# yjxiong/action-detection

Measured on AMD Instinct MI355X. Metric: proposals/sec (9-seg BNInception SSN fwd+bwd), higher is better.
Workload: dtype f32

## Files before the change

action-detection_amd/_lib.py:

```python
import ctypes
import os
import subprocess
import threading

import torch

_HERE = os.path.dirname(os.path.abspath(__file__))
CSRC = os.path.join(_HERE, "csrc")
LIB_PATH = os.path.join(_HERE, "libssn_hip.so")
SOURCES = ["conv_igemm.hip", "conv_x6.hip", "conv_x6_rect.hip", "conv_wgrad.hip", "conv_wgrad_x6.hip", "elementwise.hip", "bn_train.hip", "frames.hip", "detect.hip", "detect_batch.hip", "pool.hip", "stpp.hip", "heads_losses.hip", "conv_pl.hip", "planes_ops.hip", "planes_bn.hip", "wgrad_pl.hip", "tag.hip", "eval.hip", "actionness.hip", "train_step.hip", "flow.hip", "jpeg.hip", "jpeg_encode.hip", "jpeg_transcode.hip", "jpeg_roundtrip.hip", "video_cls.hip", "proposal_list.hip", "proposal_text.hip", "proposal_eval.hip", "test_table.hip"]

STPP_MAX_PARTS = 24


class SsnStppTable(ctypes.Structure):
    _fields_ = [("n_parts", ctypes.c_int), ("n_seg", ctypes.c_int),
                ("act_lo", ctypes.c_int), ("act_hi", ctypes.c_int),
                ("lo", ctypes.c_int * STPP_MAX_PARTS), ("hi", ctypes.c_int * STPP_MAX_PARTS),
                ("norm", ctypes.c_int * STPP_MAX_PARTS), ("col", ctypes.c_int * STPP_MAX_PARTS)]


_SIGS = {
    "ssn_conv_bn_relu_fwd": "pppppiiiiliiiliiiiipp",
    "ssn_bn_fold": "pppppfppip",
    "ssn_relu_bn_bwd": "pppiiillpp",
    "ssn_conv_dgrad": "pppiiiiliiiliiiiplpiipp",
    "ssn_conv_pack_weights": "ppiiiip",
    "ssn_conv_pack_weights_multi": "ippppppppp",
    "ssn_conv_wgrad": "ppppiiiiliiiliiiplip",
    "ssn_conv_wgrad_x6": "ppppiiiililiiiplippiipp",
    "ssn_wgrad_reduce": "pppiiip",
    "ssn_wgrad_reduce_taps": "pppiiiip",
    "ssn_conv_x6_pack_weights_multi": "ippppppppppppp",
    "ssn_conv_x6_fwd": "pppppiiiiliiiliiiiiippiiipp",
    "ssn_conv_x6_dgrad": "pppiiiiliiiliiiplpiippiipp",
    "ssn_conv_x6_fwd_rect": "pppppiiiiliiiliiiiiiippp",
    "ssn_conv_x6_pack_dgrad_s2": "ppiip",
    "ssn_conv_x6_dgrad_s2": "pppiiiiliiiliplpiippip",
    "ssn_conv_x6_pack_dgrad_rect": "ppiiiip",
    "ssn_conv_x6_pack_rect_multi": "ipppppppp",
    "ssn_conv_x6_dgrad_rect": "pppiiiililiiiiiplpiippp",
    "ssn_conv_wgrad_x6_rect": "ppppiiiililiiiiiplippp",
    "ssn_conv_x6_pack_weights_rect": "ppiiiip",
# ... 75 lines not shown
    "ssn_row_scatter": "pppiiip",
    "ssn_ce_loss_fwd": "ppppiip",
    "ssn_ce_loss_bwd": "pppppiip",
    "ssn_completeness_loss_fwd": "pppppiiiiiifp",
    "ssn_completeness_loss_bwd": "ppppiifp",
    "ssn_cw_smoothl1_fwd": "pppppiip",
    "ssn_total_loss_fwd": "ppiippiiiiiifpppiiffpppppp",
    "ssn_total_loss_bwd": "ppiipiifpiiffpppppppp",
    "ssn_label_select": "pppipipippppp",
    "ssn_param_checksum": "pipppip",
    "ssn_cw_smoothl1_bwd": "ppppiip",
    "ssn_sgd_step": "ppplffffipp",
    "ssn_sgd_step_multi": "ippppppffipp",
    "ssn_bn_fold_multi": "ipppppppppp",
    "ssn_sumsq": "plpipp",
    "ssn_step_meters": "plpiipidppp",
    "ssn_sumsq_multi": "ippplffpp",
    "ssn_sgd_step_multi_dev": "ippppppfpipp",
    "ssn_scale": "plpfp",
    "ssn_add_inplace": "pplp",
    "ssn_embed_planes": "ppiiiiliilp",
    "ssn_space_to_depth2": "ppiiiipp",
    "ssn_s2d_weights": "ppiiip",
    "ssn_s2d_weights_bwd": "ppiiip",
    "ssn_pl_scales_update": "pppiiiip",
    "ssn_pl_range_check": "pppiip",
    "ssn_pl_from_f32": "plppiiiilippp",
    "ssn_pl_to_f32": "pplpliiipp",
    "ssn_pl_im2col": "pplppliiiiiiiiiiip",
    "ssn_conv_pl_fwd": "pppppppiiiiliiiliiiiiiipppiiip",
    "ssn_conv_pl_dgrad": "pppppiiiiliiiliiiiiplpipppiiip",
    "ssn_conv_wgrad_pl": "ppppppiiiiliiiliiiiiplippiipp",
    "ssn_wgrad_reduce_multi": "ipppppppp",
    "ssn_conv_wgrad_pl_group": "ippppppppppplplp",
    "ssn_conv_wgrad_pl_group_lanes": "ippppppppppplplp" + "pii",
    "ssn_conv_pl_dgrad_s2": "pppppiiiiliiiliiplpipppp",
    "ssn_pl_maxpool_fwd": "pplpplpiiiiiiiiipppp",
    "ssn_pl_maxpool_bwd": "pplpppl" + "i" * 10 + "plpipppplp",
    "ssn_pl_avgpool_affine": "pplpplppiiiiiiipppp",
    "ssn_pl_relu_bn_bwd": "pplplpiiippp",
    "ssn_pl_gap_fwd": "pplpiiipp",
    "ssn_pl_gap_bwd": "pppliiiplpppp",
    "ssn_pl_channel_sum": "pplpiiipplp",
    "ssn_pl_channel_sum_multi": "ippppipppplp",
    "ssn_conv_x6_pack_batch_begin": "",
    "ssn_conv_x6_pack_batch_end": "plip",
    "ssn_conv_x6_pack_batch_end_lanes": "pliipp",
    "ssn_conv_x6_pack_batch_join": "p",
    "ssn_pl_bn_train_stats": "pplpppppp" + "iiiffplp",
    "ssn_pl_bn_train_apply": "pplppplpp" + "ppppiiiip",
    "ssn_pl_bn_train_bwd": "pplpplpplp" + "ppppp" + "pplpp" + "pliiiplp",
}
_CT = {"p": ctypes.c_void_p, "i": ctypes.c_int, "l": ctypes.c_long, "f": ctypes.c_float, "d": ctypes.c_double,
       "u": ctypes.c_ulonglong}

EXPORTS = sorted(list(_SIGS) + ["ssn_last_error", "ssn_abi_version", "ssn_conv_wgrad_workspace_bytes",
                                "ssn_conv_pick_tile", "ssn_conv_packed_floats", "ssn_conv_x6_packed_floats", "ssn_conv_x6_packed_floats_rect", "ssn_conv_x6_packed_floats_dgrad_rect", "ssn_conv_wgrad_x6_rect_workspace_bytes", "ssn_conv_x6_dgrad_s2_packed_floats", "ssn_conv_x6_debug_flags", "ssn_conv_x6_debug_trace",
                                "ssn_conv_wgrad_x6_workspace_bytes", "ssn_detections_workspace_bytes", "ssn_detections_batch_workspace_bytes",
                                "ssn_conv_debug_flags", "ssn_channel_sum_shares", "ssn_bn_train_workspace_floats",
                                "ssn_conv_dgrad_layout", "ssn_conv_pl_tiles", "ssn_conv_pl_halo_taken", "ssn_conv_pl_debug_flags", "ssn_conv_pl_debug_trace", "ssn_conv_wgrad_pl_debug_trace", "ssn_conv_wgrad_pl_debug_flags", "ssn_conv_pl_tile_shape", "ssn_conv_wgrad_pl_tiles", "ssn_conv_wgrad_pl_workspace_bytes", "ssn_conv_wgrad_pl_group_workspace_bytes", "ssn_conv_wgrad_pl_group_table_bytes", "ssn_conv_wgrad_pl_group_tuning", "ssn_pl_channel_sum_workspace_bytes", "ssn_pl_bn_train_workspace_bytes", "ssn_conv_x6_pack_batch_entries", "ssn_conv_x6_pack_entry_bytes", "ssn_conv_x6_pack_batch_abort", "ssn_frames_resize_workspace_bytes", "ssn_frames_scale_workspace_bytes",
                                "ssn_tag_workspace_bytes", "ssn_tag_lds_candidates", "ssn_eval_workspace_bytes", "ssn_eval_lds_gt",
                                "ssn_proposal_eval_max_points", "ssn_proposal_eval_workspace_bytes",
                                "ssn_vcls_lds_rows", "ssn_vcls_metrics_workspace_bytes",
                                "ssn_sumsq_multi_workspace_floats", "ssn_train_step_launches"])


# ... 178 lines not shown
```

action-detection_amd/csrc/wgrad_pl.hip:

```cpp
#include "planes.h"

#include <algorithm>
#include <cmath>
#include <cstdlib>
#include <map>
#include <mutex>
#include <vector>

namespace {

using namespace pl;

struct WgPlArgs {
    const void* g_hi;
    const void* g_lo;
    const void* x_hi;
    const void* x_lo;
    float* part;
    unsigned long long* trace;
    int dbg;
    const float* g_scale;
    const float* x_scale;
    int g_row_split, g_row_gap;
    int N, Cin, H, W;
// ... 484 lines not shown
        if (ci >= p.Cin) continue;
#pragma unroll
        for (int i = 0; i < TM; ++i)
#pragma unroll
            for (int r = 0; r < 16; ++r) {
                const int m = m0 + (wm * TM + i) * 32 + (r & 3) + 8 * (r >> 2) + 4 * lh;
                if (m < p.M) {
#pragma unroll
                    for (int t = 0; t < KK; ++t) out[(long)m * p.ldp + t * p.Cin + ci] = acc[t][i][j][r] * inv;
                }
            }
    }
    if (do_bias && li == 0) {
        const float ginv = 1.f / *p.g_scale;
#pragma unroll
        for (int i = 0; i < TM; ++i)
#pragma unroll
            for (int r = 0; r < 16; ++r) {
                const int m = m0 + (wm * TM + i) * 32 + (r & 3) + 8 * (r >> 2) + 4 * lh;
                if (m < p.M) out[(long)m * p.ldp + p.K] = accb[i][r] * ginv;
            }
    }
    trc.end(p);
}

template <int KK, int TM, int TC, int XP, int KG = 1>
__global__ __launch_bounds__(256 * KG, (KG > 1 || KK * TM * TC >= 18 || TM * TC >= 4) ? 1 : 2) void wgrad_pl9_kernel(WgPlArgs p) {
    __shared__ __attribute__((aligned(1024))) unsigned char lds[wgpl9_lds_bytes<TM, TC, XP>()];
    wgrad_pl9_body<KK, TM, TC, XP, KG>(p, blockIdx.x, lds);
}


constexpr int WGG_MAX = 96;
constexpr int WGG_WRITE = 12;
struct WgGroupEntry {
    WgPlArgs a;
    int variant;
    uint32_t nblk;
};
struct WgGroupIndex {
    int count;
    int blk0[WGG_MAX + 1];
};
struct WgGroupChunk {
    WgGroupEntry e[WGG_WRITE];
    int count;
};
__global__ __launch_bounds__(64) void wgrad_group_write_kernel(WgGroupChunk c, WgGroupEntry* table, int first) {
    if ((int)threadIdx.x < c.count) table[first + threadIdx.x] = c.e[threadIdx.x];
}
__device__ __forceinline__ int group_problem_of_block(const WgGroupIndex& ix, int b) {
    int lo = 0, hi = ix.count - 1;
    while (lo < hi) {
        const int mid = (lo + hi + 1) >> 1;
        if (ix.blk0[mid] <= b) lo = mid; else hi = mid - 1;
    }
    return wave_uniform(lo);
}

template <int XP, int KG, int KH = 3, int KW = 3>
__global__ __launch_bounds__(256 * KG, KG > 1 ? 1 : 2) void wgrad_group9_kernel(const WgGroupEntry* __restrict__ table, WgGroupIndex ix) {
    __shared__ __attribute__((aligned(1024))) unsigned char lds[wgpl9_lds_bytes<1, 1, XP>()];
    const int e = group_problem_of_block(ix, (int)blockIdx.x);
    const uint32_t bid = blockIdx.x - (uint32_t)ix.blk0[e];
    const auto* ent = SSN_CONST_PTR(WgGroupEntry, table) + e;
    if (bid >= ent->nblk) return;
    const WgPlArgs p = ent->a;
    wgrad_pl9_body<KH * KW, 1, 1, XP, KG, KH, KW, KH / 2, KW / 2>(p, bid, lds);
}

constexpr int WGG1_LDS = 65536;
static_assert(wgpl_lds_dwords<2, 2, 2, 2>() * 4 <= WGG1_LDS && wgpl_lds_dwords<1, 4, 3, 1>() * 4 <= WGG1_LDS &&
              wgpl_lds_dwords<2, 2, 1, 1>() * 4 <= WGG1_LDS && wgpl9_lds_bytes<1, 1, 4>() <= WGG1_LDS, "group LDS");
__global__ __launch_bounds__(256, 2) void wgrad_group1_kernel(const WgGroupEntry* __restrict__ table, WgGroupIndex ix) {
    __shared__ __attribute__((aligned(1024))) unsigned char lds[WGG1_LDS];
    const int e = group_problem_of_block(ix, (int)blockIdx.x);
    const uint32_t bid = blockIdx.x - (uint32_t)ix.blk0[e];
    const auto* ent = SSN_CONST_PTR(WgGroupEntry, table) + e;
    if (bid >= ent->nblk) return;
    const WgPlArgs p = ent->a;
// ... 631 lines not shown
    for (WgGroupItem& it : items) {
        it.ws_off = off;
        off += ((long)it.a.splits * it.kg * it.a.M * it.a.ldp * (long)sizeof(float) + 1023) / 1024 * 1024;
    }
    *ws_total = off;
    return SSN_OK;
}
}

extern "C" void ssn_conv_wgrad_pl_group_tuning(double fixed_nine, double fixed_one, int min_units_nine, int min_units_one) {
    if (fixed_nine > 0) g_group_fixed[0] = fixed_nine;
    if (fixed_one > 0) g_group_fixed[1] = fixed_one;
    if (min_units_nine > 0) g_group_min_units[0] = min_units_nine;
    if (min_units_one > 0) g_group_min_units[1] = min_units_one;
}
extern "C" long ssn_conv_wgrad_pl_group_table_bytes(int count) { return (long)(count > 0 ? count : 1) * (long)sizeof(WgGroupEntry); }

extern "C" long ssn_conv_wgrad_pl_group_workspace_bytes(int count, const int* shape, const long* groups, int* plan_out) {
    if (count <= 0 || !shape || !groups) return 0;
    std::vector<WgGroupItem> items;
    long total = 0;
    if (plan_group_all(count, shape, groups, nullptr, nullptr, nullptr, nullptr, nullptr, nullptr, nullptr, nullptr, items, &total) != SSN_OK)
        return -1;
    if (plan_out)
        for (int i = 0; i < count; ++i) {
            plan_out[i * 4] = items[(size_t)i].family;
            plan_out[i * 4 + 1] = items[(size_t)i].variant;
            plan_out[i * 4 + 2] = items[(size_t)i].a.splits;
            plan_out[i * 4 + 3] = items[(size_t)i].a.ksteps_per_split;
        }
    return total;
}

extern "C" int ssn_wgrad_reduce_multi(int count, const float* const* part, float* const* dw, float* const* db, const int* M,
                                      const int* K, const int* splits, const int* taps, hipStream_t stream);

namespace {
constexpr int WGL_MAX = 8;
#if defined(__HIP__)
struct WgLaneEvents {
    hipEvent_t fork;
    hipEvent_t join[WGL_MAX];
};
WgLaneEvents* wgrad_lane_events(hipStream_t stream) {
    static std::mutex mu;
    static std::map<int, WgLaneEvents> cache;
    std::lock_guard<std::mutex> lock(mu);
    int dev = 0;
    if (hipGetDevice(&dev) != hipSuccess) return nullptr;
    auto it = cache.find(dev);
    if (it != cache.end()) return &it->second;
    hipStreamCaptureStatus status = hipStreamCaptureStatusNone;
    if (hipStreamIsCapturing(stream, &status) != hipSuccess || status != hipStreamCaptureStatusNone) {
        (void)hipGetLastError();
        return nullptr;
    }
    WgLaneEvents ev;
    bool ok = hipEventCreateWithFlags(&ev.fork, hipEventDisableTiming) == hipSuccess;
    for (int k = 0; k < WGL_MAX && ok; ++k) ok = hipEventCreateWithFlags(&ev.join[k], hipEventDisableTiming) == hipSuccess;
    if (!ok) {
        (void)hipGetLastError();
        return nullptr;
    }
    return &cache.emplace(dev, ev).first->second;
}
#endif

int wgrad_group_run(int count, const void* const* g_hi, const void* const* g_lo, const void* const* x_hi, const void* const* x_lo,
// ... 41 lines not shown
                return ((double)x->a.M + (double)x->a.Cin * s2) / ((double)x->a.M * x->a.Cin * x->a.kh * x->a.kw);
            };
            std::stable_sort(fam.begin(), fam.end(), [&](const WgGroupItem* x, const WgGroupItem* y) { return bytes_per_mac(x) > bytes_per_mac(y); });
            std::vector<WgGroupItem*> dealt;
            for (size_t lo = 0, hi = fam.size(); lo < hi;) {
                dealt.push_back(fam[lo++]);
                if (lo < hi) dealt.push_back(fam[--hi]);
            }
            fam.swap(dealt);
        }
        for (size_t base = 0; base < fam.size(); base += WGG_MAX) {
            const int n = (int)std::min<size_t>(WGG_MAX, fam.size() - base);
            Launch L;
            L.family = f;
            L.first = first;
            L.items.assign(fam.begin() + (long)base, fam.begin() + (long)base + n);
            L.slab_bytes = 0;
            for (const WgGroupItem* it : L.items) L.slab_bytes += (long)it->a.splits * it->kg * it->a.M * it->a.ldp * (long)sizeof(float);
            launches.push_back(std::move(L));
            first += n;
        }
    }
    if (per_family)
        std::stable_sort(launches.begin(), launches.end(), [](const Launch& x, const Launch& y) { return x.slab_bytes > y.slab_bytes; });

    int fan = n_lanes;
#if defined(__HIP__)
    WgLaneEvents* ev = fan > 0 ? wgrad_lane_events(stream) : nullptr;
    if (!ev) fan = 0;
#else
    SSN_CHECK_ARG(n_lanes == 0, "conv wgrad pl group: the host build has no streams");
#endif

    auto write_table = [&](const Launch& L, WgGroupIndex& ix) -> long {
        const int n = (int)L.items.size();
        ix.count = n;
        long blocks = 0;
        for (int c0 = 0; c0 < n; c0 += WGG_WRITE) {
            WgGroupChunk ch;
            ch.count = std::min(WGG_WRITE, n - c0);
            for (int j = 0; j < ch.count; ++j) {
                WgGroupItem& it = *L.items[(size_t)(c0 + j)];
                it.a.part = reinterpret_cast<float*>(static_cast<char*>(workspace) + it.ws_off);
                ch.e[j].a = it.a;
                ch.e[j].variant = it.variant;
                ch.e[j].nblk = (uint32_t)(it.tiles * it.a.splits);
                ix.blk0[c0 + j] = (int)blocks;
                blocks += (it.tiles * it.a.splits + 7) / 8 * 8;
            }
            hipLaunchKernelGGL(wgrad_group_write_kernel, dim3(1), dim3(64), 0, stream, ch, dev, L.first + c0);
        }
        for (int j = n; j <= WGG_MAX; ++j) ix.blk0[j] = (int)blocks;
        return blocks;
    };
    auto launch_family = [&](const Launch& L, const WgGroupIndex& ix, long blocks, hipStream_t s) {
        const WgGroupEntry* tab = dev + L.first;
        switch (L.family) {
            case WGF_9_XP6: hipLaunchKernelGGL((wgrad_group9_kernel<6, 1>), dim3((unsigned)blocks), dim3(256), 0, s, tab, ix); break;
            case WGF_9_XP8: hipLaunchKernelGGL((wgrad_group9_kernel<8, 2>), dim3((unsigned)blocks), dim3(512), 0, s, tab, ix); break;
            case WGF_9_XP12: hipLaunchKernelGGL((wgrad_group9_kernel<12, 2>), dim3((unsigned)blocks), dim3(512), 0, s, tab, ix); break;
            case WGF_STEM: hipLaunchKernelGGL(wgrad_group_stem_kernel, dim3((unsigned)blocks), dim3(512), 0, s, tab, ix); break;
            case WGF_7_ROW: hipLaunchKernelGGL((wgrad_group9_kernel<6, 1, 1, 7>), dim3((unsigned)blocks), dim3(256), 0, s, tab, ix); break;
            case WGF_7_COL: hipLaunchKernelGGL((wgrad_group9_kernel<12, 2, 7, 1>), dim3((unsigned)blocks), dim3(512), 0, s, tab, ix); break;
            default: hipLaunchKernelGGL(wgrad_group1_kernel, dim3((unsigned)blocks), dim3(256), 0, s, tab, ix); break;
        }
    };
    auto reduce = [&](const std::vector<const WgGroupItem*>& its, hipStream_t s) -> int {
        const size_t n = its.size();
        std::vector<const float*> parts(n);
        std::vector<float*> dws(n), dbs(n);
        std::vector<int> Ms(n), Ks(n), sp(n), tp(n);
        for (size_t i = 0; i < n; ++i) {
            const WgGroupItem& it = *its[i];
            parts[i] = reinterpret_cast<const float*>(static_cast<char*>(workspace) + it.ws_off);
            dws[i] = it.dw;
            dbs[i] = it.db;
            Ms[i] = it.a.M;
            Ks[i] = it.a.K;
            sp[i] = it.a.splits * it.kg;
            tp[i] = it.taps;
        }
        return ssn_wgrad_reduce_multi((int)n, parts.data(), dws.data(), dbs.data(), Ms.data(), Ks.data(), sp.data(), tp.data(), s);
    };

    std::vector<WgGroupIndex> index(launches.size());
    std::vector<long> grid(launches.size());
    if (fan > 0) {
        for (size_t k = 0; k < launches.size(); ++k) {
            grid[k] = write_table(launches[k], index[k]);
            SSN_CHECK_ARG(grid[k] < (1l << 31), "conv wgrad pl group: too many blocks");
        }
        SSN_CHECK_LAUNCH("conv_wgrad_pl_group");
    }
#if defined(__HIP__)
    if (fan > 0) {
        bool ok = hipEventRecord(ev->fork, stream) == hipSuccess;
        for (int k = 0; k < fan && ok; ++k) ok = hipStreamWaitEvent(lanes[k], ev->fork, 0) == hipSuccess;
        if (!ok) {
            ssn_set_error("conv wgrad pl group: fork of the side streams failed: %s", hipGetErrorString(hipGetLastError()));
            return SSN_ERR_LAUNCH;
        }
    }
#endif
    for (size_t k = 0; k < launches.size(); ++k) {
        const Launch& L = launches[k];
        hipStream_t s = fan > 0 ? lanes[k % (size_t)fan] : stream;
        if (fan == 0) {
            grid[k] = write_table(L, index[k]);
            SSN_CHECK_ARG(grid[k] < (1l << 31), "conv wgrad pl group: too many blocks");
        }
        launch_family(L, index[k], grid[k], s);
        if (per_family) {
            SSN_CHECK_LAUNCH("conv_wgrad_pl_group");
            rc = reduce(std::vector<const WgGroupItem*>(L.items.begin(), L.items.end()), s);
            if (rc != SSN_OK) break;
        }
    }
#if defined(__HIP__)
    if (fan > 0 && join) {
        bool ok = true;
        for (int k = 0; k < fan; ++k) {
            ok = hipEventRecord(ev->join[k], lanes[k]) == hipSuccess && ok;
            ok = hipStreamWaitEvent(stream, ev->join[k], 0) == hipSuccess && ok;
        }
        if (!ok && rc == SSN_OK) {
            ssn_set_error("conv wgrad pl group: join of the side streams failed: %s", hipGetErrorString(hipGetLastError()));
            return SSN_ERR_LAUNCH;
        }
    }
#endif
    if (rc != SSN_OK) return rc;
    SSN_CHECK_LAUNCH("conv_wgrad_pl_group");
    if (per_family) return SSN_OK;
    std::vector<const WgGroupItem*> all((size_t)count);
    for (int i = 0; i < count; ++i) all[(size_t)i] = &items[(size_t)i];
    return reduce(all, stream);
}
}

extern "C" int ssn_conv_wgrad_pl_group(int count, const void* const* g_hi, const void* const* g_lo, const void* const* x_hi,
                                       const void* const* x_lo, float* const* dw, float* const* db, const int* shape,
// ... 86 lines not shown
```

action-detection_amd/planes.py:

```python
import torch

from . import _lib
from . import kernels as K
from .kernels import _p, _stream


class SlotPool:

    def __init__(self, n, device, flag=None):
        self.device = device
        self.amax = torch.zeros(n, device=device, dtype=torch.float32)
        self.scale = torch.ones(n, device=device, dtype=torch.float32)
        self.flag = torch.zeros(2, device=device, dtype=torch.int32) if flag is None else flag
        self.used = 0
        self.odd_extra_bits = 0

    def take(self):
        i = self.used
        if i >= self.amax.numel():
            raise RuntimeError("slot pool exhausted")
        self.used += 1
        return i

    def update(self, exact=False, first=0, count=None):
# ... 158 lines not shown
             mask.groups if mask is not None else 0, _p(mask_scale), tile_cfg, dy.t.scale_ptr, dx.t.scale_ptr, dx.t.amax_ptr,
             int(k_split), int(k_gap), int(bool(taps_reversed)), _st(lib, dy.t))


def wgrad_workspace_bytes(n, cin, cout, ho, wo, kh, kw, tile_cfg=-1):
    return int(_lib.get_lib().cdll.ssn_conv_wgrad_pl_workspace_bytes(n, cin, cout, ho, wo, kh, kw, tile_cfg))


def conv_wgrad(g, x, dw, db, kh, kw, stride, pad_h, pad_w, workspace, tile_cfg=-1, cin=None, g_row_split=0, g_row_gap=0, defer=None):
    import ctypes
    lib = _lib_for(g.t)
    h, w = x.hw
    ho, wo = g.hw
    cin = x.c if cin is None else cin
    info = (ctypes.c_int * 2)() if defer is not None else None
    lib.call("ssn_conv_wgrad_pl", g.hi, g.lo, x.hi, x.lo, _p(dw), _p(db), x.n, cin, h, w, x.groups, g.c, ho, wo, g.groups, kh, kw,
             stride, pad_h, pad_w, _p(workspace), workspace.numel() * workspace.element_size(), tile_cfg, g.t.scale_ptr,
             x.t.scale_ptr, int(g_row_split), int(g_row_gap), ctypes.addressof(info) if info is not None else None, _st(lib, g.t))
    if defer is not None:
        defer.append((workspace, dw, db, g.c, cin * kh * kw, int(info[0]), int(info[1])))


def wgrad_reduce_multi(entries):
    import ctypes
    if not entries:
        return
    lib = _lib.get_lib()
    n = len(entries)
    parts = (ctypes.c_void_p * n)(*[e[0].data_ptr() for e in entries])
    dws = (ctypes.c_void_p * n)(*[e[1].data_ptr() for e in entries])
    dbs = (ctypes.c_void_p * n)(*[(e[2].data_ptr() if e[2] is not None else None) for e in entries])
    arr = [(ctypes.c_int * n)(*[int(e[k]) for e in entries]) for k in (3, 4, 5, 6)]
    lib.call("ssn_wgrad_reduce_multi", n, ctypes.addressof(parts), ctypes.addressof(dws), ctypes.addressof(dbs),
             ctypes.addressof(arr[0]), ctypes.addressof(arr[1]), ctypes.addressof(arr[2]), ctypes.addressof(arr[3]),
             _stream(lib, entries[0][0]))


class WgradJob:

    __slots__ = ("g", "x", "dw", "db", "kh", "kw", "stride", "pad_h", "pad_w", "cin", "g_row_split", "g_row_gap", "hint", "units")

    def __init__(self, g, x, dw, db, kh, kw, stride, pad_h, pad_w, cin=None, g_row_split=0, g_row_gap=0, hint=-1, units=0):
        self.g, self.x, self.dw, self.db = g, x, dw, db
        self.kh, self.kw, self.stride, self.pad_h, self.pad_w = int(kh), int(kw), int(stride), int(pad_h), int(pad_w)
        self.cin = x.c if cin is None else int(cin)
        self.g_row_split, self.g_row_gap, self.hint = int(g_row_split), int(g_row_gap), int(hint)
        self.units = int(units)

    def shape16(self):
        h, w = self.x.hw
        ho, wo = self.g.hw
        return [self.x.n, self.cin, h, w, self.g.c, ho, wo, self.kh, self.kw, self.stride, self.pad_h, self.pad_w,
                self.g_row_split, self.g_row_gap, self.hint, self.units]


def _wgrad_group_arrays(jobs):
    import ctypes
    n = len(jobs)
    shape = (ctypes.c_int * (16 * n))(*[v for j in jobs for v in j.shape16()])
    groups = (ctypes.c_long * (2 * n))(*[v for j in jobs for v in (j.x.groups, j.g.groups)])
    return shape, groups


def wgrad_group_plan(jobs):
    import ctypes
    lib = _lib.get_lib()
# ... 182 lines not shown
```

action-detection_amd/planes_exec.py:

```python
import contextlib
import itertools
import math

import torch

from . import kernels as K
from . import planes as P
from .planes import PSlice, PlaneTensor


class PlanesState:

    MAX_TENSORS = 512
    GRAD_EXTRA_BITS = 3

    def __init__(self, device, flag=None):
        self.pool = P.SlotPool(2 * self.MAX_TENSORS, device, flag)
        self.pool.odd_extra_bits = self.GRAD_EXTRA_BITS
        self.act_slot = {}
        self.grad_slot = {}
        self.fwd_calibrated = False
        self.bwd_calibrated = False
        self.calibration_passes = [0, 0]
        self.recalibrations = [0, 0]
# ... 447 lines not shown
            ws_bytes = max(ws_bytes, need)
        else:
            ws_off[op["lids"][0]] = (ws_bytes, need)
            ws_bytes += need
    ws_all = net._workspace(ws_bytes, dev)

    def ws_of(op):
        if op["lids"][0] not in ws_off:
            return None
        o, nb = ws_off[op["lids"][0]]
        return ws_all[o // 4:(o + nb) // 4]
    cs_ws = torch.empty(P.channel_sum_workspace_bytes(sum(op["cout"] for op in plan if op["kind"] == "conv" and
                                                           (op.get("raw") or "raw_from" in op)) + 8) // 4,
                        device=dev, dtype=torch.float32)

    dg_s2 = {op["lids"][0]: _dgrad_is_s2(op) for op in plan if op["kind"] == "conv" and op["src"] != "data"}
    packed_dg = extras["packed_dg"]

    def src_key(op):
        return (op["src"], op.get("src_c0", 0))
    last_writer = {}
    for idx in range(len(plan) - 1, -1, -1):
        last_writer[src_key(plan[idx])] = idx
    first_conv = net._conv_ids[0]
    stem_out = None
    for op in plan:
        if op["kind"] == "conv" and op.get("s2d") and "data_s2d_f32" in acts:
            readers = [q for q in plan if q.get("src") == op["dst"]]
            if len(readers) == 1 and readers[0]["kind"] == "pool" and readers[0]["pool"] == "max" and op["dst_c0"] == 0:
                stem_out = op["dst"]

    conv_of = {op["dst"]: op for op in plan if op["kind"] == "conv" and op.get("bn_train")}

    def launch_all(grads, fire_hook):
        masked, inited = {}, set()
        pending_end = total
        pending_reduce, pending_sums = [], []

        pending_wgrad = []
        wgrad_flops_total = sum(2.0 * n * shapes[q["dst"]][1] * shapes[q["dst"]][2] * q["cout"] * q["cin"] * _conv_taps(q)[0] * _conv_taps(q)[1]
                                for q in plan if q["kind"] == "conv")
        pending_post = []

        if not (net.wgrad_lanes and net.group_wgrad):
            wl_streams = None
        elif dfeat.is_cuda and net.overlap_wgrad and net.branch_lanes:
            cur = torch.cuda.current_stream(dev).cuda_stream
            wl_streams = [s for s in net._wgrad_streams(dev, 3) if s.cuda_stream != cur]
        else:
            wl_streams = []

        def flush():
            if pending_wgrad:
                jobs = [j for j, _ in pending_wgrad]
                net._timed("conv_wgrad_pl", "group", sum(f for _, f in pending_wgrad),
                           lambda: P.conv_wgrad_group(jobs, *net._wgrad_group_buffers(jobs, dev), streams=wl_streams))
            if pending_reduce:
                entries = list(pending_reduce)
                net._timed("conv_wgrad_pl", "reduce_multi", 0.0, lambda: P.wgrad_reduce_multi(entries))
            if pending_sums:
                P.channel_sum_multi(list(pending_sums), cs_ws)
            for fn in pending_post:
                fn()
            del pending_reduce[:], pending_sums[:], pending_wgrad[:], pending_post[:]
        group = net.group_wgrad
        defer = pending_reduce if net.defer_wgrad_reduce else None

# ... 169 lines not shown
                        net._timed("conv_dgrad_pl", lids[0], flops,
                                   lambda: P.conv_dgrad_s2(gs, wt, dx, op["p"], acc_flag, tcfg, mask=my, mask_scale=ms))
                    else:
                        net._timed("conv_dgrad_pl", lids[0], flops, lambda: P.conv_dgrad(
                            gs, wt, dx, kh, kw, ph, pw, acc_flag, tcfg, mask=my, mask_scale=ms, k_split=op.get("row_split", 0),
                            k_gap=op.get("row_gap", 0), taps_reversed=op["rect"]))
                    inited.add(key)
                closes_block = (lids[0].endswith("_1x1") or lids[0] == first_conv
                                or lids[0] in ("inception_3c_3x3_reduce", "inception_4e_3x3_reduce"))
                if fire_hook and net.grad_ready_hook is not None and closes_block:
                    if not (group and pending_wgrad) or sum(f for _, f in pending_wgrad) >= wgrad_flops_total / 3.0 or wo == 0:
                        flush()
                        net.grad_ready_hook.range_ready(flat, wo, pending_end)
                        pending_end = wo

        side_ops, joins = _branch_lanes(plan) if (net.branch_lanes and dfeat.is_cuda) else ({}, set())
        side = net._side_stream(dev) if side_ops else None
        main = torch.cuda.current_stream(dev) if side_ops else None
        forks_bwd = {i + 3 for i, kind in side_ops.items() if kind == "fork"}
        joins_bwd = {i - 1 for i, kind in side_ops.items() if kind == "fork"}
        for idx in range(len(plan) - 1, -1, -1):
            if idx in joins_bwd:
                main.wait_stream(side)
            if idx in side_ops:
                gbuf(plan[idx]["src"])
                if idx in forks_bwd:
                    side.wait_stream(main)
                with torch.cuda.stream(side):
                    run_op(idx)
            else:
                run_op(idx)
        if side_ops:
            main.wait_stream(side)
        flush()
        if fire_hook and net.grad_ready_hook is not None:
            if pending_end > 0:
                net.grad_ready_hook.range_ready(flat, 0, pending_end)
            net.grad_ready_hook.finish()

    grads = {}
    hook_obj = net.grad_ready_hook if hook else None
    overlapping = hook_obj is not None and not getattr(hook_obj, "deferred", False)
    capturing = _capturing(dfeat)
    polling = net.scale_guard == "sync" and not capturing
    refire = False

    def silent_pass():
        launch_all(grads, False)

    st.nonfinite = False
    if not st.bwd_calibrated:
        if capturing:
            raise RuntimeError("planes executor: the first backward of a state calibrates its scales with host syncs and cannot "
                               "be captured into a hipGraph; run one eager step first")
        amax0 = float(dfeat.abs().max().item())
        if not math.isfinite(amax0):
            amax0 = 0.0
        hw = 1
        for op in plan:
            if op["kind"] == "gap":
                hw = shapes[op["src"]][1] * shapes[op["src"]][2]
        s0 = 2.0 ** math.floor(math.log2(2048.0 / max(amax0 / hw, 1e-30))) if amax0 > 0 else 1.0
        st.pool.scale[1::2] = s0
        silent_pass()
        st.calibration_passes[1] = 1 + st.settle(silent_pass, "gradient")
        st.bwd_calibrated = True
        refire = overlapping
    else:
        launch_all(grads, overlapping)
        if net.scale_guard != "off":
            st.check()
            local = bool(st.fault()) if polling else False
            fault = local
            if polling and overlapping and hasattr(hook_obj, "agree"):
                fault = hook_obj.agree(local)
            if local:
                st.describe_fault("backward")
            if fault:
                repeats = st.settle(silent_pass, "gradient")
                st.recalibrations[1] += (1 if local else 0) + repeats
                refire = overlapping
    if hook_obj is not None:
        if refire:
            launch_all(grads, True)
        elif not overlapping:
            hook_obj.range_ready(flat, 0, total)
            hook_obj.finish()
    if st.nonfinite or extras.get("nonfinite"):
        st.pool.flag[0] = 1
        flat.fill_(float("nan"))
        for dg, db_ in bn_grads.values():
            dg.fill_(float("nan"))
            db_.fill_(float("nan"))
    out = []
    for lid in net._conv_ids:
        conv = getattr(net, lid)
        wo, wn, bo, bn = lay[lid]
        out.append(flat[wo:wo + wn].view_as(conv.weight) if conv.weight.requires_grad else None)
        out.append(flat[bo:bo + bn] if conv.bias.requires_grad else None)
    for lid in net._train_bn_ids():
        bnm = getattr(net, lid + "_bn")
        dgamma, dbeta = bn_grads[lid]
        out.append(dgamma if bnm.weight.requires_grad else None)
        out.append(dbeta if bnm.bias.requires_grad else None)
# ... 29 lines not shown
```

include/ssn_hip.h:

```cpp
#ifndef SSN_HIP_H
#define SSN_HIP_H

#include <stddef.h>

#ifdef __cplusplus
extern "C" {
#endif

typedef struct ihipStream_t* hipStream_t;

#define SSN_ERR_ARG (-1)
#define SSN_ERR_LAUNCH (-2)
#define SSN_ERR_WORKSPACE (-3)

const char* ssn_last_error(void);
int ssn_abi_version(void);

long ssn_conv_packed_floats(int Cout, int Cin, int ksize, int transposed);
int ssn_conv_pack_weights(const float* w, float* packed, int Cout, int Cin, int ksize, int transposed,
                          hipStream_t stream);

int ssn_conv_pack_weights_multi(int count, const float* const* w0, const float* const* w1, float* const* out,
                                const int* cout, const int* cin, const int* ksize, const int* mode, const int* split,
                                hipStream_t stream);
// ... 312 lines not shown
int ssn_s2d_weights(const float* w, float* w2, int Cout, int C, int k, hipStream_t stream);
int ssn_s2d_weights_bwd(const float* dw2, float* dw, int Cout, int C, int k, hipStream_t stream);
int ssn_add_inplace(float* dst, const float* src, long n, hipStream_t stream);
int ssn_embed_planes(const float* g, float* out, int N, int C, int Ho, int Wo, long g_img_stride, int H, int W,
                     long out_img_stride, hipStream_t stream);

int ssn_pl_scales_update(float* amax, float* scale, int* flag, int n, int exact, int slot0, int odd_extra_bits, hipStream_t stream);
int ssn_pl_range_check(const float* amax, const float* scale, int* flag, int n, int odd_extra_bits, hipStream_t stream);
int ssn_pl_from_f32(const float* x, long x_img_stride, void* hi, void* lo, int N, int C, int H, int W, long img_groups, int s2d,
                    const float* scale, float* amax, hipStream_t stream);
int ssn_pl_im2col(const void* x_hi, const void* x_lo, long x_img_groups, void* y_hi, void* y_lo, long y_img_groups, int N, int C, int H,
                  int W, int Ho, int Wo, int kh, int kw, int stride, int pad_h, int pad_w, hipStream_t stream);
int ssn_pl_to_f32(const void* hi, const void* lo, long img_groups, float* y, long y_img_stride, int N, int C, int HW,
                  const float* scale, hipStream_t stream);
int ssn_conv_pl_fwd(const void* x_hi, const void* x_lo, const float* w_packed, const float* scale, const float* shift, void* y_hi,
                    void* y_lo, int N, int Cin, int H, int W, long x_img_groups, int Cout, int Ho, int Wo, long y_img_groups, int kh,
                    int kw, int stride, int pad_h, int pad_w, int relu, int tile_cfg, const float* x_scale, const float* y_scale,
                    float* y_amax, int raw_from, int row_split, int row_gap, hipStream_t stream);
int ssn_conv_pl_dgrad(const void* dy_hi, const void* dy_lo, const float* wt_packed, void* dx_hi, void* dx_lo, int N, int Cout,
                      int Ho, int Wo, long dy_img_groups, int Cin, int H, int W, long dx_img_groups, int kh, int kw, int pad_h,
                      int pad_w, int accumulate, const void* mask_hi, long mask_img_groups, const float* mask_scale, int tile_cfg,
                      const float* dy_scale, const float* dx_scale, float* dx_amax, int k_split, int k_gap, int taps_reversed,
                      hipStream_t stream);
int ssn_conv_pl_dgrad_s2(const void* dy_hi, const void* dy_lo, const float* wt_packed, void* dx_hi, void* dx_lo, int N, int Cout,
                         int Ho, int Wo, long dy_img_groups, int Cin, int H, int W, long dx_img_groups, int pad, int accumulate,
                         const void* mask_hi, long mask_img_groups, const float* mask_scale, int tile_cfg, const float* dy_scale,
                         const float* dx_scale, float* dx_amax, hipStream_t stream);
int ssn_conv_wgrad_pl(const void* g_hi, const void* g_lo, const void* x_hi, const void* x_lo, float* dw, float* db, int N, int Cin,
                      int H, int W, long x_img_groups, int Cout, int Ho, int Wo, long g_img_groups, int kh, int kw, int stride,
                      int pad_h, int pad_w, void* workspace, long ws_bytes, int tile_cfg, const float* g_scale,
                      const float* x_scale, int g_row_split, int g_row_gap, int* deferred_reduce, hipStream_t stream);
int ssn_wgrad_reduce_multi(int count, const float* const* part, float* const* dw, float* const* db, const int* M, const int* K,
                           const int* splits, const int* taps, hipStream_t stream);
long ssn_conv_wgrad_pl_workspace_bytes(int N, int Cin, int Cout, int Ho, int Wo, int kh, int kw, int tile_cfg);
int ssn_conv_wgrad_pl_group(int count, const void* const* g_hi, const void* const* g_lo, const void* const* x_hi,
                            const void* const* x_lo, float* const* dw, float* const* db, const int* shape, const long* groups,
                            const float* const* g_scale, const float* const* x_scale, void* workspace, long ws_bytes, void* table,
                            long table_bytes, hipStream_t stream);
int ssn_conv_wgrad_pl_group_lanes(int count, const void* const* g_hi, const void* const* g_lo, const void* const* x_hi,
                                  const void* const* x_lo, float* const* dw, float* const* db, const int* shape, const long* groups,
                                  const float* const* g_scale, const float* const* x_scale, void* workspace, long ws_bytes,
                                  void* table, long table_bytes, hipStream_t stream, const hipStream_t* lanes, int n_lanes, int join);
long ssn_conv_wgrad_pl_group_workspace_bytes(int count, const int* shape, const long* groups, int* plan_out);
long ssn_conv_wgrad_pl_group_table_bytes(int count);
void ssn_conv_wgrad_pl_group_tuning(double fixed_nine, double fixed_one, int min_units_nine, int min_units_one);
int ssn_conv_wgrad_pl_tiles(void);
int ssn_conv_pl_tiles(void);
int ssn_conv_pl_halo_taken(int N, int H, int W, int tile_cfg);
int ssn_conv_pl_tile_shape(int cfg, int* bm, int* bn);
void ssn_conv_pl_debug_flags(int flags);
void ssn_conv_pl_debug_trace(unsigned long long* buf);
void ssn_conv_wgrad_pl_debug_trace(unsigned long long* buf);
void ssn_conv_wgrad_pl_debug_flags(int flags);
int ssn_pl_maxpool_fwd(const void* x_hi, const void* x_lo, long x_img_groups, void* y_hi, void* y_lo, long y_img_groups,
                       unsigned char* argmax, int N, int C, int H, int W, int Ho, int Wo, int k, int s, int pad,
                       const float* x_scale, const float* y_scale, float* y_amax, hipStream_t stream);
int ssn_pl_maxpool_bwd(const void* dy_hi, const void* dy_lo, long dy_img_groups, const unsigned char* argmax, void* dx_hi,
                       void* dx_lo, long dx_img_groups, int N, int C, int H, int W, int Ho, int Wo, int k, int s, int pad,
                       int accumulate, const void* mask_hi, long mask_img_groups, const float* mask_scale, int mask_pooled,
                       const float* dy_scale, const float* dx_scale, float* dx_amax, float* dx_f32, long dx_f32_img_stride,
                       hipStream_t stream);
int ssn_pl_avgpool_affine(const void* x_hi, const void* x_lo, long x_img_groups, void* y_hi, void* y_lo, long y_img_groups,
                          const float* scale, const float* shift, int relu, int N, int C, int H, int W, int k, int pad,
                          const float* x_scale, const float* y_scale, float* y_amax, hipStream_t stream);
int ssn_pl_relu_bn_bwd(void* g_hi, void* g_lo, long g_img_groups, const void* y_hi, long y_img_groups, const float* scale, int N,
                       int C, int HW, const float* g_scale, float* g_amax, hipStream_t stream);
// ... 71 lines not shown
```

Measured before the change: 2408.

## Add LDS-staged ordered wgrad split-K reduction and move plan writes onto lanes

Adds a new split-K reduction kernel for weight gradients. Each workgroup owns a strip of output columns, stages batches of split partials through LDS with coalesced (optionally 16-byte) loads, and sums them in fixed order. The strip width is chosen per problem size. The grouped wgrad path now calls this kernel instead of the old reduce_multi, and writes its plan tables on the side lanes after the fork instead of on the main stream before it. The chunk size for table writes also grows, and the scale-guard check moves to just before the final flush. These changes aim to cut reduction bandwidth cost and serial launch overhead, at the risk of more LDS traffic and extra synchronisation inside the reduction.

```diff
diff --git a/action-detection_amd/_lib.py b/action-detection_amd/_lib.py
--- a/action-detection_amd/_lib.py
+++ b/action-detection_amd/_lib.py
@@ -8,7 +8,7 @@
 _HERE = os.path.dirname(os.path.abspath(__file__))
 CSRC = os.path.join(_HERE, "csrc")
 LIB_PATH = os.path.join(_HERE, "libssn_hip.so")
-SOURCES = ["conv_igemm.hip", "conv_x6.hip", "conv_x6_rect.hip", "conv_wgrad.hip", "conv_wgrad_x6.hip", "elementwise.hip", "bn_train.hip", "frames.hip", "detect.hip", "detect_batch.hip", "pool.hip", "stpp.hip", "heads_losses.hip", "conv_pl.hip", "planes_ops.hip", "planes_bn.hip", "wgrad_pl.hip", "tag.hip", "eval.hip", "actionness.hip", "train_step.hip", "flow.hip", "jpeg.hip", "jpeg_encode.hip", "jpeg_transcode.hip", "jpeg_roundtrip.hip", "video_cls.hip", "proposal_list.hip", "proposal_text.hip", "proposal_eval.hip", "test_table.hip"]
+SOURCES = ["conv_igemm.hip", "conv_x6.hip", "conv_x6_rect.hip", "conv_wgrad.hip", "conv_wgrad_x6.hip", "elementwise.hip", "bn_train.hip", "frames.hip", "detect.hip", "detect_batch.hip", "pool.hip", "stpp.hip", "heads_losses.hip", "conv_pl.hip", "planes_ops.hip", "planes_bn.hip", "wgrad_pl.hip", "wgrad_sum.hip", "tag.hip", "eval.hip", "actionness.hip", "train_step.hip", "flow.hip", "jpeg.hip", "jpeg_encode.hip", "jpeg_transcode.hip", "jpeg_roundtrip.hip", "video_cls.hip", "proposal_list.hip", "proposal_text.hip", "proposal_eval.hip", "test_table.hip"]
 
 STPP_MAX_PARTS = 24
 
@@ -150,6 +150,7 @@
     "ssn_conv_pl_dgrad": "pppppiiiiliiiliiiiiplpipppiiip",
     "ssn_conv_wgrad_pl": "ppppppiiiiliiiliiiiiplippiipp",
     "ssn_wgrad_reduce_multi": "ipppppppp",
+    "ssn_wgrad_sum_ordered": "ipppppppp",
     "ssn_conv_wgrad_pl_group": "ippppppppppplplp",
     "ssn_conv_wgrad_pl_group_lanes": "ippppppppppplplp" + "pii",
     "ssn_conv_pl_dgrad_s2": "pppppiiiiliiiliiplpipppp",
diff --git a/action-detection_amd/csrc/wgrad_pl.hip b/action-detection_amd/csrc/wgrad_pl.hip
--- a/action-detection_amd/csrc/wgrad_pl.hip
+++ b/action-detection_amd/csrc/wgrad_pl.hip
@@ -540,7 +540,7 @@
 
 
 constexpr int WGG_MAX = 96;
-constexpr int WGG_WRITE = 12;
+constexpr int WGG_WRITE = 15;
 struct WgGroupEntry {
     WgPlArgs a;
     int variant;
@@ -554,6 +554,7 @@
     WgGroupEntry e[WGG_WRITE];
     int count;
 };
+static_assert(sizeof(WgGroupChunk) + sizeof(WgGroupEntry*) + sizeof(int) <= 4096, "plan-write kernel arguments");
 __global__ __launch_bounds__(64) void wgrad_group_write_kernel(WgGroupChunk c, WgGroupEntry* table, int first) {
     if ((int)threadIdx.x < c.count) table[first + threadIdx.x] = c.e[threadIdx.x];
 }
@@ -1251,8 +1252,8 @@
     return total;
 }
 
-extern "C" int ssn_wgrad_reduce_multi(int count, const float* const* part, float* const* dw, float* const* db, const int* M,
-                                      const int* K, const int* splits, const int* taps, hipStream_t stream);
+extern "C" int ssn_wgrad_sum_ordered(int count, const float* const* part, float* const* dw, float* const* db, const int* M,
+                                     const int* K, const int* splits, const int* taps, hipStream_t stream);
 
 namespace {
 constexpr int WGL_MAX = 8;
@@ -1360,7 +1361,7 @@
     SSN_CHECK_ARG(n_lanes == 0, "conv wgrad pl group: the host build has no streams");
 #endif
 
-    auto write_table = [&](const Launch& L, WgGroupIndex& ix) -> long {
+    auto write_table = [&](const Launch& L, WgGroupIndex& ix, hipStream_t ws) -> long {
         const int n = (int)L.items.size();
         ix.count = n;
         long blocks = 0;
@@ -1376,7 +1377,7 @@
                 ix.blk0[c0 + j] = (int)blocks;
                 blocks += (it.tiles * it.a.splits + 7) / 8 * 8;
             }
-            hipLaunchKernelGGL(wgrad_group_write_kernel, dim3(1), dim3(64), 0, stream, ch, dev, L.first + c0);
+            hipLaunchKernelGGL(wgrad_group_write_kernel, dim3(1), dim3(64), 0, ws, ch, dev, L.first + c0);
         }
         for (int j = n; j <= WGG_MAX; ++j) ix.blk0[j] = (int)blocks;
         return blocks;
@@ -1408,18 +1409,11 @@
             sp[i] = it.a.splits * it.kg;
             tp[i] = it.taps;
         }
-        return ssn_wgrad_reduce_multi((int)n, parts.data(), dws.data(), dbs.data(), Ms.data(), Ks.data(), sp.data(), tp.data(), s);
+        return ssn_wgrad_sum_ordered((int)n, parts.data(), dws.data(), dbs.data(), Ms.data(), Ks.data(), sp.data(), tp.data(), s);
     };
 
     std::vector<WgGroupIndex> index(launches.size());
     std::vector<long> grid(launches.size());
-    if (fan > 0) {
-        for (size_t k = 0; k < launches.size(); ++k) {
-            grid[k] = write_table(launches[k], index[k]);
-            SSN_CHECK_ARG(grid[k] < (1l << 31), "conv wgrad pl group: too many blocks");
-        }
-        SSN_CHECK_LAUNCH("conv_wgrad_pl_group");
-    }
 #if defined(__HIP__)
     if (fan > 0) {
         bool ok = hipEventRecord(ev->fork, stream) == hipSuccess;
@@ -1428,13 +1422,19 @@
             ssn_set_error("conv wgrad pl group: fork of the side streams failed: %s", hipGetErrorString(hipGetLastError()));
             return SSN_ERR_LAUNCH;
         }
+        for (size_t k = 0; k < launches.size(); ++k) grid[k] = write_table(launches[k], index[k], lanes[k % (size_t)fan]);
+        for (size_t k = 0; k < launches.size() && rc == SSN_OK; ++k)
+            if (grid[k] >= (1l << 31)) {
+                ssn_set_error("conv wgrad pl group: too many blocks");
+                rc = SSN_ERR_ARG;
+            }
     }
 #endif
-    for (size_t k = 0; k < launches.size(); ++k) {
+    for (size_t k = 0; k < launches.size() && rc == SSN_OK; ++k) {
         const Launch& L = launches[k];
         hipStream_t s = fan > 0 ? lanes[k % (size_t)fan] : stream;
         if (fan == 0) {
-            grid[k] = write_table(L, index[k]);
+            grid[k] = write_table(L, index[k], stream);
             SSN_CHECK_ARG(grid[k] < (1l << 31), "conv wgrad pl group: too many blocks");
         }
         launch_family(L, index[k], grid[k], s);
diff --git a/action-detection_amd/csrc/wgrad_sum.hip b/action-detection_amd/csrc/wgrad_sum.hip
--- /dev/null
+++ b/action-detection_amd/csrc/wgrad_sum.hip
@@ -0,0 +1,163 @@
+#include <vector>
+
+#include "ssn_common.h"
+
+namespace {
+
+constexpr int WS_MAX = 48;
+constexpr int WS_THREADS = 256;
+constexpr int WS_U = 8;
+constexpr int WS_LDS_FLOATS = WS_THREADS * WS_U * 4;
+constexpr int WS_WIDE = 256, WS_NARROW = 64;
+constexpr long WS_COVER = 512;
+
+struct SumTable {
+    const float* part[WS_MAX];
+    float* dw[WS_MAX];
+    float* db[WS_MAX];
+    int M[WS_MAX], K[WS_MAX], splits[WS_MAX], taps[WS_MAX];
+    int mode[WS_MAX];
+    int blk0[WS_MAX + 1];
+    int count;
+};
+
+template <int W, bool VEC>
+__device__ __forceinline__ void wgrad_sum_strip(const float* __restrict__ part, float* __restrict__ dw, float* __restrict__ db, int M,
+                                                int K, int splits, int taps, uint32_t strip, float* lds) {
+    constexpr int Q = W / 4;
+    constexpr int ZW = WS_THREADS / Q;
+    constexpr int ZB = ZW * WS_U;
+    static_assert(ZB * W == WS_LDS_FLOATS, "batch size");
+    const int t = (int)threadIdx.x;
+    const int quad = t % Q, zway = t / Q;
+    const uint32_t ldp = (uint32_t)K + 1u;
+    const uint32_t total = (uint32_t)M * ldp;
+    const uint32_t idx0 = strip * (uint32_t)W;
+    uint32_t e[4];
+    bool in[4];
+#pragma unroll
+    for (int j = 0; j < 4; ++j) {
+        e[j] = VEC ? (uint32_t)(quad * 4 + j) : (uint32_t)(j * Q + quad);
+        in[j] = idx0 + e[j] < total;
+    }
+    f32x4 v[WS_U];
+#pragma unroll
+    for (int q = 0; q < WS_U; ++q) v[q] = f32x4{0.f, 0.f, 0.f, 0.f};
+    auto fetch = [&](int zb) {
+#pragma unroll
+        for (int q = 0; q < WS_U; ++q) {
+            const int z = zb + q * ZW + zway;
+            if (z >= splits) continue;
+            const float* src = part + (long)z * total + idx0;
+            if (VEC) {
+                if (in[0]) v[q] = *reinterpret_cast<const f32x4*>(src + e[0]);
+            } else {
+#pragma unroll
+                for (int j = 0; j < 4; ++j)
+                    if (in[j]) v[q][j] = src[e[j]];
+            }
+        }
+    };
+    auto stage = [&](int zb) {
+#pragma unroll
+        for (int q = 0; q < WS_U; ++q) {
+            const int row = q * ZW + zway;
+            if (zb + row >= splits) continue;
+            float* dst = lds + row * W;
+            if (VEC) {
+                if (in[0]) *reinterpret_cast<f32x4*>(dst + e[0]) = v[q];
+            } else {
+#pragma unroll
+                for (int j = 0; j < 4; ++j)
+                    if (in[j]) dst[e[j]] = v[q][j];
+            }
+        }
+    };
+    const uint32_t idx = idx0 + (uint32_t)t;
+    const bool owner = t < W && idx < total;
+    float s = 0.f;
+    fetch(0);
+    for (int zb = 0; zb < splits; zb += ZB) {
+        stage(zb);
+        __syncthreads();
+        if (zb + ZB < splits) fetch(zb + ZB);
+        if (owner) {
+            const int rows = splits - zb < ZB ? splits - zb : ZB;
+            const float* col = lds + t;
+#pragma unroll 8
+            for (int r = 0; r < rows; ++r) s += col[r * W];
+        }
+        __syncthreads();
+    }
+    if (!owner) return;
+    const int m = (int)(idx / ldp);
+    const int kk = (int)(idx - (uint32_t)m * ldp);
+    if (kk < K) {
+        int col = kk;
+        if (taps > 1) {
+            const int cin = K / taps, tt = kk / cin;
+            col = (kk - tt * cin) * taps + tt;
+        }
+        dw[(long)m * K + col] = s;
+    } else if (db) {
+        db[m] = s;
+    }
+}
+
+__global__ __launch_bounds__(WS_THREADS) void wgrad_sum_ordered_kernel(SumTable tb) {
+    __shared__ __attribute__((aligned(16))) float lds[WS_LDS_FLOATS];
+    int lo = 0, hi = tb.count - 1;
+    while (lo < hi) {
+        const int mid = (lo + hi + 1) >> 1;
+        if (tb.blk0[mid] <= (int)blockIdx.x) lo = mid; else hi = mid - 1;
+    }
+    const int ti = wave_uniform(lo);
+    const uint32_t strip = blockIdx.x - (uint32_t)tb.blk0[ti];
+    const float* part = tb.part[ti];
+    float* dw = tb.dw[ti];
+    float* db = tb.db[ti];
+    const int M = tb.M[ti], K = tb.K[ti], splits = tb.splits[ti], taps = tb.taps[ti];
+    switch (wave_uniform(tb.mode[ti])) {
+        case 0: wgrad_sum_strip<WS_WIDE, false>(part, dw, db, M, K, splits, taps, strip, lds); break;
+        case 1: wgrad_sum_strip<WS_WIDE, true>(part, dw, db, M, K, splits, taps, strip, lds); break;
+        case 2: wgrad_sum_strip<WS_NARROW, false>(part, dw, db, M, K, splits, taps, strip, lds); break;
+        default: wgrad_sum_strip<WS_NARROW, true>(part, dw, db, M, K, splits, taps, strip, lds); break;
+    }
+}
+
+}
+
+extern "C" int ssn_wgrad_sum_ordered(int count, const float* const* part, float* const* dw, float* const* db, const int* M,
+                                     const int* K, const int* splits, const int* taps, hipStream_t stream) {
+    SSN_CHECK_ARG(count >= 0 && (count == 0 || (part && dw && db && M && K && splits && taps)), "wgrad sum ordered: bad arguments");
+    for (int base = 0; base < count; base += WS_MAX) {
+        SumTable t;
+        t.count = count - base < WS_MAX ? count - base : WS_MAX;
+        long blocks = 0;
+        for (int i = 0; i < t.count; ++i) {
+            const int j = base + i;
+            SSN_CHECK_ARG(part[j] && dw[j] && M[j] > 0 && K[j] > 0 && splits[j] > 0 && taps[j] >= 1 && K[j] % taps[j] == 0 &&
+                              (long)M[j] * (K[j] + 1) < (1l << 31),
+                          "wgrad sum ordered: bad entry %d", j);
+            const long total = (long)M[j] * (K[j] + 1);
+            const bool vec = total % 4 == 0 && (reinterpret_cast<uintptr_t>(part[j]) & 15) == 0;
+            const bool narrow = (total + WS_WIDE - 1) / WS_WIDE < WS_COVER;
+            const int W = narrow ? WS_NARROW : WS_WIDE;
+            t.part[i] = part[j];
+            t.dw[i] = dw[j];
+            t.db[i] = db[j];
+            t.M[i] = M[j];
+            t.K[i] = K[j];
+            t.splits[i] = splits[j];
+            t.taps[i] = taps[j];
+            t.mode[i] = (vec ? 1 : 0) | (narrow ? 2 : 0);
+            t.blk0[i] = (int)blocks;
+            blocks += (total + W - 1) / W;
+            SSN_CHECK_ARG(blocks < (1l << 31), "wgrad sum ordered: too many workgroups");
+        }
+        for (int i = t.count; i <= WS_MAX; ++i) t.blk0[i] = (int)blocks;
+        hipLaunchKernelGGL(wgrad_sum_ordered_kernel, dim3((unsigned)blocks), dim3(WS_THREADS), 0, stream, t);
+    }
+    SSN_CHECK_LAUNCH("wgrad_sum_ordered");
+    return SSN_OK;
+}
diff --git a/action-detection_amd/planes.py b/action-detection_amd/planes.py
--- a/action-detection_amd/planes.py
+++ b/action-detection_amd/planes.py
@@ -214,6 +214,21 @@
     dbs = (ctypes.c_void_p * n)(*[(e[2].data_ptr() if e[2] is not None else None) for e in entries])
     arr = [(ctypes.c_int * n)(*[int(e[k]) for e in entries]) for k in (3, 4, 5, 6)]
     lib.call("ssn_wgrad_reduce_multi", n, ctypes.addressof(parts), ctypes.addressof(dws), ctypes.addressof(dbs),
+             ctypes.addressof(arr[0]), ctypes.addressof(arr[1]), ctypes.addressof(arr[2]), ctypes.addressof(arr[3]),
+             _stream(lib, entries[0][0]))
+
+
+def wgrad_sum_ordered(entries):
+    import ctypes
+    if not entries:
+        return
+    lib = _lib.get_lib()
+    n = len(entries)
+    parts = (ctypes.c_void_p * n)(*[e[0].data_ptr() for e in entries])
+    dws = (ctypes.c_void_p * n)(*[e[1].data_ptr() for e in entries])
+    dbs = (ctypes.c_void_p * n)(*[(e[2].data_ptr() if e[2] is not None else None) for e in entries])
+    arr = [(ctypes.c_int * n)(*[int(e[k]) for e in entries]) for k in (3, 4, 5, 6)]
+    lib.call("ssn_wgrad_sum_ordered", n, ctypes.addressof(parts), ctypes.addressof(dws), ctypes.addressof(dbs),
              ctypes.addressof(arr[0]), ctypes.addressof(arr[1]), ctypes.addressof(arr[2]), ctypes.addressof(arr[3]),
              _stream(lib, entries[0][0]))
 
diff --git a/action-detection_amd/planes_exec.py b/action-detection_amd/planes_exec.py
--- a/action-detection_amd/planes_exec.py
+++ b/action-detection_amd/planes_exec.py
@@ -503,7 +503,7 @@
 
     conv_of = {op["dst"]: op for op in plan if op["kind"] == "conv" and op.get("bn_train")}
 
-    def launch_all(grads, fire_hook):
+    def launch_all(grads, fire_hook, before_last_flush=None):
         masked, inited = {}, set()
         pending_end = total
         pending_reduce, pending_sums = [], []
@@ -739,6 +739,8 @@
                 run_op(idx)
         if side_ops:
             main.wait_stream(side)
+        if before_last_flush is not None:
+            before_last_flush()
         flush()
         if fire_hook and net.grad_ready_hook is not None:
             if pending_end > 0:
@@ -774,9 +776,8 @@
         st.bwd_calibrated = True
         refire = overlapping
     else:
-        launch_all(grads, overlapping)
+        launch_all(grads, overlapping, st.check if net.scale_guard != "off" else None)
         if net.scale_guard != "off":
-            st.check()
             local = bool(st.fault()) if polling else False
             fault = local
             if polling and overlapping and hasattr(hook_obj, "agree"):
diff --git a/include/ssn_hip.h b/include/ssn_hip.h
--- a/include/ssn_hip.h
+++ b/include/ssn_hip.h
@@ -368,6 +368,8 @@
                       const float* x_scale, int g_row_split, int g_row_gap, int* deferred_reduce, hipStream_t stream);
 int ssn_wgrad_reduce_multi(int count, const float* const* part, float* const* dw, float* const* db, const int* M, const int* K,
                            const int* splits, const int* taps, hipStream_t stream);
+int ssn_wgrad_sum_ordered(int count, const float* const* part, float* const* dw, float* const* db, const int* M, const int* K,
+                          const int* splits, const int* taps, hipStream_t stream);
 long ssn_conv_wgrad_pl_workspace_bytes(int N, int Cin, int Cout, int Ho, int Wo, int kh, int kw, int tile_cfg);
 int ssn_conv_wgrad_pl_group(int count, const void* const* g_hi, const void* const* g_lo, const void* const* x_hi,
                             const void* const* x_lo, float* const* dw, float* const* db, const int* shape, const long* groups,
```

Result: no change. 2426, median of 3 (+0.7%).
